# sz3/libcimbar

Hardware: NVIDIA H100
Metric: decoded cimbar frames/sec (1024x1024 mode-B) (higher is better)
Workload: dtype u8 (integer/bitwise; float32 only in the colour classifier, bit-exact vs reference)

## Files before the change

libcimbar_b200/csrc/k2_rs.cu:

```cuda
#include "cb200_common.cuh"
#include "k2_rs.cuh"
#include <cstring>
#include <cstdint>

namespace cb200 {

constexpr int kMaxParity = 64;

__constant__ uint8_t c_gf_exp[512];
__constant__ uint8_t c_gf_log[256];

__device__ __forceinline__ uint32_t slot_value(const uint8_t* __restrict__ cells, const uint16_t* __restrict__ idx,
                                               uint32_t s, int stream, int symbol_bits)
{
    uint32_t v = cells[idx[s]] & 0x7Fu;
    uint32_t sym_mask = (1u << symbol_bits) - 1u;
    if (stream == 0) return v & sym_mask;
    if (stream == 1) return v >> symbol_bits;
    return v;
}

__device__ __forceinline__ uint32_t stream_byte(const uint8_t* __restrict__ cells, const uint16_t* __restrict__ idx,
                                                uint32_t B, int w, int stream, int symbol_bits, uint32_t nslots)
{
    uint32_t bit0 = 8u * B;
    uint32_t s = bit0 / (uint32_t)w;
    uint32_t skip = bit0 - s * (uint32_t)w;
    uint32_t acc = 0, nbits = 0;
    while (nbits < skip + 8u) {
        uint32_t v = (s < nslots) ? slot_value(cells, idx, s, stream, symbol_bits) : 0u;
        acc = (acc << w) | v;
        nbits += (uint32_t)w;
        ++s;
    }
    return (acc >> (nbits - skip - 8u)) & 0xFFu;
}

__global__ void __launch_bounds__(256)
k_pack_raw(const Mode m, const uint8_t* __restrict__ cellvals, const uint16_t* __restrict__ idx, int n_frames,
           uint8_t* __restrict__ raw)
{
    int B = blockIdx.x * blockDim.x + threadIdx.x;
    int f = blockIdx.y;
    if (B >= m.cap_all || f >= n_frames) return;
    const uint8_t* cells = cellvals + (size_t)f * m.num_cells;
    uint32_t v;
    if (m.legacy) v = stream_byte(cells, idx, (uint32_t)B, m.symbol_bits + m.color_bits, 2, m.symbol_bits, (uint32_t)m.num_cells);
    else if (B < m.cap_sym) v = stream_byte(cells, idx, (uint32_t)B, m.symbol_bits, 0, m.symbol_bits, (uint32_t)m.num_cells);
    else v = stream_byte(cells, idx, (uint32_t)(B - m.cap_sym), m.color_bits, 1, m.symbol_bits, (uint32_t)m.num_cells);
    raw[(size_t)f * m.cap_all + B] = (uint8_t)v;
}

constexpr int kRsWarpsPerCta = 16;
constexpr int kLaDim = 40;
constexpr int kStagePitch = 196;

template <int T>
struct RsSmem {
    static constexpr bool kSynTable = false;
    static constexpr int GL = 8 * T;
    static constexpr int G = 32 / GL;
    uint8_t exp[512];
    uint8_t log[256];
    struct PerWarp {
        alignas(16) uint8_t stage[G * kStagePitch];
        alignas(4) uint8_t rem[64];
        alignas(2) uint16_t remlog[kMaxParity];
        uint8_t synd[kMaxParity];
        uint8_t loc[kMaxParity + 8];
        uint8_t last[kMaxParity + 8];
        uint8_t omega[kMaxParity];
        uint8_t roots[kMaxParity + 8];
    } w[kRsWarpsPerCta];
    uint8_t la[kLaDim][kLaDim];
};

template <class S>
__device__ __forceinline__ uint32_t gf_mul(const S& s, uint32_t a, uint32_t b)
{
    if (a == 0 || b == 0) return 0;
    return s.exp[(uint32_t)s.log[a] + (uint32_t)s.log[b]];
}
template <class S>
__device__ __forceinline__ uint32_t gf_div(const S& s, uint32_t a, uint32_t b)
{
    if (a == 0 || b == 0) return 0;
    return s.exp[255u + (uint32_t)s.log[a] - (uint32_t)s.log[b]];
}
__device__ __forceinline__ uint32_t lds_u32(uint32_t shared_addr)
{
    uint32_t v;
    asm("ld.shared.u32 %0, [%1];" : "=r"(v) : "r"(shared_addr));
    return v;
}
__device__ __forceinline__ uint32_t warp_xor(uint32_t v)
{
#pragma unroll
    for (int o = 16; o > 0; o >>= 1) v ^= __shfl_xor_sync(0xffffffffu, v, o);
    return v;
}

template <int T, class S, class W>
__device__ __forceinline__ bool rs_correct_block(const S& s, W& w, uint8_t* enc, const int md, const int blk, const int pad,
                                                 const bool holds, const uint32_t word, const int k, const int lane)
{
            __syncwarp();
            if (holds) reinterpret_cast<uint32_t*>(w.rem)[k] = word;
            __syncwarp();
            if constexpr (S::kSynTable) {
                if (lane < md) {
                    const uint32_t rb = w.rem[pad + lane];
                    w.masks[lane] = make_uint2((((rb & 15u) * 0x00204081u) & 0x01010101u) * 0xFFu, (((rb >> 4) * 0x00204081u) & 0x01010101u) * 0xFFu);
                }
                __syncwarp();
                uint32_t ax = 0, ay = 0;
#pragma unroll 6
                for (int i = 0; i < md; ++i) {
                    const uint2 mk = w.masks[i];
                    const uint2 tw = s.wsyn[i][lane];
                    ax ^= tw.x & mk.x; ay ^= tw.y & mk.y;
                }
                uint32_t x = ax ^ ay;
                x ^= x >> 16; x ^= x >> 8;
                if (lane < md) w.synd[lane] = (uint8_t)x;
            } else {
            for (int i = lane; i < md; i += 32) { const uint32_t rb = w.rem[pad + i]; w.remlog[i] = (uint16_t)(rb | ((uint32_t)s.log[rb] << 8)); }
            __syncwarp();
#pragma unroll
            for (int q = 0; q < T; ++q) {
                const int j = lane + 32 * q;
                if (j < md) {
                    uint32_t acc = 0;
#pragma unroll 6
                    for (int i = 0; i < md; ++i) {
                        const uint32_t rl = w.remlog[i];
                        const uint32_t t = s.exp[(rl >> 8) + (uint32_t)s.la[i][j]];
                        acc ^= (rl & 0xFFu) ? t : 0u;
                    }
                    w.synd[j] = (uint8_t)acc;
                }
            }
            }
            __syncwarp();
        uint32_t numerrors = 0, loc_order = 0, last_order = 0, last_disc = 1, delay = 1;
        if (T == 1) {
            uint32_t loc = (lane == 0), last = (lane == 0), lloc = 0;
            const uint32_t syn = (lane < md) ? (uint32_t)w.synd[lane] : 0u;
            const uint32_t spk = syn | ((uint32_t)s.log[syn] << 8);
            for (uint32_t i = 0; i < (uint32_t)md; ++i) {
                const uint32_t p = __shfl_sync(0xffffffffu, spk, (int)(i - (uint32_t)lane) & 31);
                uint32_t term = 0;
                if ((uint32_t)lane <= numerrors && loc != 0 && (p & 0xFFu) != 0) term = s.exp[lloc + (p >> 8)];
                const uint32_t disc = __reduce_xor_sync(0xffffffffu, term);
                if (disc == 0) { delay++; continue; }
                const uint32_t lscale = 255u + (uint32_t)s.log[disc] - (uint32_t)s.log[last_disc];
                const uint32_t top = last_order + delay;
                const uint32_t shifted = __shfl_up_sync(0xffffffffu, last, delay);
                const uint32_t lsc = lscale >= 255u ? lscale - 255u : lscale;
                const uint32_t sh = ((uint32_t)lane >= delay && (uint32_t)lane <= top && shifted != 0) ? (uint32_t)s.exp[(uint32_t)s.log[shifted] + lsc] : 0u;
                if (2 * numerrors <= i) {
                    if ((uint32_t)lane <= top) { const uint32_t t0 = loc; loc ^= sh; last = t0; }
                    lloc = s.log[loc];
                    const uint32_t tmp = loc_order;
                    loc_order = top; last_order = tmp;
                    numerrors = i + 1 - numerrors;
                    last_disc = disc;
                    delay = 1;
                    continue;
                }
                loc ^= sh;
                lloc = s.log[loc];
                if (top > loc_order) loc_order = top;
                delay++;
            }
            w.loc[lane] = (uint8_t)loc;
            if (lane < 8) w.loc[32 + lane] = 0;
            __syncwarp();
        } else {
        for (int j = lane; j < kMaxParity + 8; j += 32) { w.loc[j] = (j == 0); w.last[j] = (j == 0); }
        __syncwarp();
        for (uint32_t i = 0; i < (uint32_t)md; ++i) {
            uint32_t part = 0;
            for (uint32_t j = 1 + lane; j <= numerrors; j += 32) part ^= gf_mul(s, w.loc[j], w.synd[i - j]);
            uint32_t disc = warp_xor(part) ^ w.synd[i];
            if (disc == 0) { delay++; continue; }
            if (2 * numerrors <= i) {
                uint32_t top = last_order + delay;
                uint32_t sh[3], lc[3];
                int q = 0;
                for (uint32_t j = lane; j <= top; j += 32, ++q) {
                    sh[q] = (j < delay) ? 0u : gf_div(s, gf_mul(s, w.last[j - delay], disc), last_disc);
                    lc[q] = w.loc[j];
                }
                __syncwarp();
                q = 0;
                for (uint32_t j = lane; j <= top; j += 32, ++q) {
                    w.loc[j] = (uint8_t)(lc[q] ^ sh[q]);
                    w.last[j] = (uint8_t)lc[q];
                }
                __syncwarp();
                uint32_t tmp = loc_order;
                loc_order = top; last_order = tmp;
                numerrors = i + 1 - numerrors;
                last_disc = disc;
                delay = 1;
                continue;
            }
            for (uint32_t j = lane; j <= last_order; j += 32)
                w.loc[j + delay] ^= (uint8_t)gf_div(s, gf_mul(s, w.last[j], disc), last_disc);
            __syncwarp();
            if (last_order + delay > loc_order) loc_order = last_order + delay;
            delay++;
        }
        }
        const uint32_t order = loc_order;

        uint32_t myroots = 0;
        for (int k = 0; k < 8; ++k) {
            uint32_t e = (uint32_t)lane * 8u + (uint32_t)k;
            if (e == 0) continue;
            uint32_t le = s.log[e];
            uint32_t acc = w.loc[order];
            for (int i = (int)order - 1; i >= 0; --i) {
                uint32_t t = acc ? (uint32_t)s.exp[(uint32_t)s.log[acc] + le] : 0u;
                acc = t ^ w.loc[i];
            }
            if (acc == 0) myroots |= 1u << k;
        }
        uint32_t cnt = __popc(myroots);
        uint32_t incl = cnt;
#pragma unroll
        for (int o = 1; o < 32; o <<= 1) { uint32_t v = __shfl_up_sync(0xffffffffu, incl, o); if (lane >= o) incl += v; }
        uint32_t total = __shfl_sync(0xffffffffu, incl, 31);
        if (total != order || order == 0) {
            if (order == 0 && total == 0) {
            }
            return false;
        }
        {
            uint32_t pos = incl - cnt;
            for (int k = 0; k < 8; ++k) if (myroots & (1u << k)) w.roots[pos++] = (uint8_t)(lane * 8 + k);
        }
        for (int k = lane; k < md; k += 32) {
            uint32_t acc = 0;
            int lim = (int)order < k ? (int)order : k;
            for (int i = 0; i <= lim; ++i) acc ^= gf_mul(s, w.loc[i], w.synd[k - i]);
            w.omega[k] = (uint8_t)acc;
        }
        __syncwarp();
        for (uint32_t q = 0; q < order; ++q) {
            const uint32_t X = w.roots[q];
            const uint32_t lx = s.log[X];
            uint32_t tn = 0, td = 0;
#pragma unroll
            for (int qq = 0; qq < T; ++qq) {
                const uint32_t i = (uint32_t)lane + 32u * (uint32_t)qq;
                const uint32_t ex = (i * lx) % 255u;
                if (i < (uint32_t)md) { const uint32_t o = w.omega[i]; if (o) tn ^= s.exp[(uint32_t)s.log[o] + ex]; }
                if (i < order && (i & 1u) == 0u) { const uint32_t c = w.loc[i + 1]; if (c) td ^= s.exp[(uint32_t)s.log[c] + ex]; }
            }
            const uint32_t num = __reduce_xor_sync(0xffffffffu, tn), den = __reduce_xor_sync(0xffffffffu, td);
            const uint32_t err = gf_div(s, num, den);
            const uint32_t inv = s.exp[510u - lx];
            const uint32_t location = s.log[inv];
            if (lane == 0 && location >= (uint32_t)md && location < (uint32_t)blk)
                enc[blk - 1 - (int)location] ^= (uint8_t)err;
        }
        __syncwarp();
        return true;
}

template <int T, bool FUSED>
__global__ void __launch_bounds__(kRsWarpsPerCta * 32, (T == 1 ? 4 : 2))
k_rs_decode(const Mode m, const uint8_t* __restrict__ raw, const uint8_t* __restrict__ cellvals, const uint16_t* __restrict__ idx,
            int n_frames, int b_begin, int b_count, uint8_t* __restrict__ data_out, uint8_t* __restrict__ block_ok,
            const uint8_t* __restrict__ rho)
{
    using Smem = RsSmem<T>;
    constexpr int GL = Smem::GL, G = Smem::G;
    extern __shared__ __align__(16) uint8_t rs_smem_raw[];
    Smem& s = *reinterpret_cast<Smem*>(rs_smem_raw);
    uint32_t* lt = reinterpret_cast<uint32_t*>(rs_smem_raw + ((sizeof(Smem) + 127) & ~size_t(127)));
    const int tid = threadIdx.x, warp = tid >> 5, lane = tid & 31;
    for (int i = tid; i < 512; i += blockDim.x) s.exp[i] = c_gf_exp[i];
    for (int i = tid; i < 256; i += blockDim.x) s.log[i] = c_gf_log[i];
    __syncthreads();
    for (int e = tid; e < m.ecc_bytes * kLaDim; e += blockDim.x) {
        const int kk = e / kLaDim, j = e % kLaDim;
        s.la[kk][j] = (uint8_t)((255 - ((j + 1) * (m.ecc_bytes - kk)) % 255) % 255);
    }
    for (int e = tid; e < 4 * 256 * GL; e += blockDim.x) {
        const int j = e / (256 * GL), v = (e / GL) & 255, k = e % GL;
        uint32_t word = 0;
#pragma unroll
        for (int bb = 0; bb < 4; ++bb) word |= gf_mul(s, (uint32_t)v, (uint32_t)rho[j * 64 + 4 * k + bb]) << (8 * bb);
        lt[e] = word;
    }
    __syncthreads();

    const int md = m.ecc_bytes, blk = m.ecc_block, msg_len = m.msg_len;
    const int Pw = (md + 3) >> 2, pad = 4 * Pw - md, lead = (4 - (blk & 3)) & 3, nsteps = (lead + blk) >> 2;
    const long total_blocks = (long)n_frames * b_count;
    const long total_units = (total_blocks + G - 1) / G;
    typename Smem::PerWarp& w = s.w[warp];
    const int grp = lane / GL, k = lane % GL;
    const uint32_t lt_lane = (uint32_t)__cvta_generic_to_shared(lt) + 4u * (uint32_t)k;
    const uint32_t stage_lane = (uint32_t)__cvta_generic_to_shared(w.stage) + (uint32_t)(grp * kStagePitch);

    for (long unit = (long)blockIdx.x * kRsWarpsPerCta + warp; unit < total_units; unit += (long)gridDim.x * kRsWarpsPerCta) {
        __syncwarp();
#pragma unroll 1
        for (int g = 0; g < G; ++g) {
            const long gb = unit * G + g;
            uint8_t* st = w.stage + g * kStagePitch;
            if (lane < lead) st[lane] = 0;
            if (gb >= total_blocks) { for (int i = lane; i < blk; i += 32) st[lead + i] = 0; continue; }
            const int f = (int)(gb / b_count), b = b_begin + (int)(gb - (long)f * b_count);
            uint8_t* enc = st + lead;
            if (FUSED) {
                const uint8_t* cells = cellvals + (size_t)f * m.num_cells;
                const bool fast = !m.legacy && m.symbol_bits == 4 && m.color_bits == 2 && blk <= 160;
                if (fast) {
                    const uint32_t B0 = (uint32_t)b * (uint32_t)blk;
                    constexpr int kU = 5;
                    if ((int)B0 < m.cap_sym) {
                        uint32_t sl[kU];
#pragma unroll
                        for (int u = 0; u < kU; ++u) {
                            const int i = lane + 32 * u;
                            sl[u] = i < blk ? *reinterpret_cast<const uint32_t*>(idx + 2u * (B0 + (uint32_t)i)) : 0u;
                        }
                        uint32_t c0[kU], c1[kU];
#pragma unroll
                        for (int u = 0; u < kU; ++u) {
                            const int i = lane + 32 * u;
                            if (i < blk) { c0[u] = cells[sl[u] & 0xFFFFu]; c1[u] = cells[sl[u] >> 16]; } else { c0[u] = c1[u] = 0; }
                        }
#pragma unroll
                        for (int u = 0; u < kU; ++u) {
                            const int i = lane + 32 * u;
                            if (i < blk) enc[i] = (uint8_t)(((c0[u] & 15u) << 4) | (c1[u] & 15u));
                        }
                    } else {
                        uint2 sl[kU];
#pragma unroll
                        for (int u = 0; u < kU; ++u) {
                            const int i = lane + 32 * u;
                            sl[u] = i < blk ? *reinterpret_cast<const uint2*>(idx + 4u * (B0 + (uint32_t)i - (uint32_t)m.cap_sym)) : make_uint2(0u, 0u);
                        }
                        uint32_t c0[kU], c1[kU], c2[kU], c3[kU];
#pragma unroll
                        for (int u = 0; u < kU; ++u) {
                            const int i = lane + 32 * u;
                            if (i < blk) { c0[u] = cells[sl[u].x & 0xFFFFu]; c1[u] = cells[sl[u].x >> 16]; c2[u] = cells[sl[u].y & 0xFFFFu]; c3[u] = cells[sl[u].y >> 16]; }
                            else { c0[u] = c1[u] = c2[u] = c3[u] = 0; }
                        }
#pragma unroll
                        for (int u = 0; u < kU; ++u) {
                            const int i = lane + 32 * u;
                            if (i < blk)
                                enc[i] = (uint8_t)((((c0[u] >> 4) & 3u) << 6) | (((c1[u] >> 4) & 3u) << 4) | (((c2[u] >> 4) & 3u) << 2) | ((c3[u] >> 4) & 3u));
                        }
                    }
                } else {
                    for (int i = lane; i < blk; i += 32) {
                        uint32_t B = (uint32_t)b * (uint32_t)blk + (uint32_t)i, v;
                        if (m.legacy) v = stream_byte(cells, idx, B, m.symbol_bits + m.color_bits, 2, m.symbol_bits, (uint32_t)m.num_cells);
                        else if ((int)B < m.cap_sym) v = stream_byte(cells, idx, B, m.symbol_bits, 0, m.symbol_bits, (uint32_t)m.num_cells);
                        else v = stream_byte(cells, idx, B - (uint32_t)m.cap_sym, m.color_bits, 1, m.symbol_bits, (uint32_t)m.num_cells);
                        enc[i] = (uint8_t)v;
                    }
                }
            } else {
                const uint8_t* enc_g = raw + (size_t)f * m.cap_all + (size_t)b * blk;
                for (int i = lane; i < blk; i += 32) enc[i] = enc_g[i];
            }
        }
        __syncwarp();

        uint32_t word = 0;
        {
            const int top_src = grp * GL + (Pw - 1);
#pragma unroll 2
            for (int t = 0; t < nsteps; ++t) {
                const uint32_t ew = lds_u32(stage_lane + 4u * (uint32_t)t);
                const uint32_t tw = __shfl_sync(0xffffffffu, word, top_src);
                const uint32_t v = tw ^ __byte_perm(ew, 0u, 0x0123);
                const uint32_t r0 = lds_u32(lt_lane + (((v) & 0xFFu) + 0u) * (4u * GL));
                const uint32_t r1 = lds_u32(lt_lane + (((v >> 8) & 0xFFu) + 256u) * (4u * GL));
                const uint32_t r2 = lds_u32(lt_lane + (((v >> 16) & 0xFFu) + 512u) * (4u * GL));
                const uint32_t r3 = lds_u32(lt_lane + ((v >> 24) + 768u) * (4u * GL));
                uint32_t prev = __shfl_up_sync(0xffffffffu, word, 1, GL);
                if (k == 0) prev = 0;
                word = prev ^ r0 ^ r1 ^ r2 ^ r3;
            }
        }
        const uint32_t dirty = __ballot_sync(0xffffffffu, k < Pw && word != 0u);

#pragma unroll 1
        for (int g = 0; g < G; ++g) {
            const long gb = unit * G + g;
            if (gb >= total_blocks) break;
            const int f = (int)(gb / b_count), b = b_begin + (int)(gb - (long)f * b_count);
            uint8_t* out = data_out + ((size_t)f * m.nblocks + b) * msg_len;
            uint8_t* enc = w.stage + g * kStagePitch + lead;
            if (((dirty >> (g * GL)) & ((1u << GL) - 1u)) == 0u) {
                for (int i = lane; i < msg_len; i += 32) out[i] = enc[i];
                if (lane == 0) block_ok[(size_t)f * m.nblocks + b] = 1;
                continue;
            }
            __syncwarp();
            const bool good = rs_correct_block<T>(s, w, enc, md, blk, pad, grp == g && k < Pw, word, k, lane);
            __syncwarp();
            if (!good) {
                for (int i = lane; i < msg_len; i += 32) out[i] = 0;
                if (lane == 0) block_ok[(size_t)f * m.nblocks + b] = 0;
                continue;
            }
        for (int i = lane; i < msg_len; i += 32) out[i] = enc[i];
        if (lane == 0) block_ok[(size_t)f * m.nblocks + b] = 1;
        }
    }
}

constexpr int kFrWarps = 32;
constexpr int kFrFrames = 2;
constexpr int kFrBlk = 155, kFrWords = 39, kFrPitch = 160;

struct RsFrSmem {
    static constexpr bool kSynTable = true;
    uint8_t exp[512];
    uint8_t log[256];
    struct PerWarp {
        alignas(8) uint2 masks[32];
        alignas(4) uint8_t rem[64];
        alignas(2) uint16_t remlog[kMaxParity];
        uint8_t synd[kMaxParity];
        uint8_t loc[kMaxParity + 8];
        uint8_t last[kMaxParity + 8];
        uint8_t omega[kMaxParity];
        uint8_t roots[kMaxParity + 8];
    } w[kFrWarps];
    uint8_t la[kLaDim][kLaDim];
    alignas(8) uint2 wsyn[32][32];
};

__device__ __forceinline__ void cp_async16(uint32_t dst_shared, const void* src)
{
    asm volatile("cp.async.cg.shared.global [%0], [%1], 16;" ::"r"(dst_shared), "l"(src) : "memory");
}

__global__ void __launch_bounds__(kFrWarps * 32, 2)
k_rs_frames(const Mode m, const uint8_t* __restrict__ cellvals, const uint16_t* __restrict__ idx, int n_frames,
            uint8_t* __restrict__ data_out, uint8_t* __restrict__ block_ok, const uint8_t* __restrict__ rho, int cell_pitch)
{
    constexpr int GL = 8, G = 4;
    extern __shared__ __align__(16) uint8_t rs_smem_raw[];
    RsFrSmem& s = *reinterpret_cast<RsFrSmem*>(rs_smem_raw);
    uint8_t* dyn = rs_smem_raw + ((sizeof(RsFrSmem) + 127) & ~size_t(127));
    uint32_t* lt = reinterpret_cast<uint32_t*>(dyn);
    uint8_t* cellbuf = dyn + sizeof(uint32_t) * 4 * 256 * GL;
    uint8_t* rows = cellbuf + (size_t)kFrFrames * cell_pitch;
    const int tid = threadIdx.x, warp = tid >> 5, lane = tid & 31;
    const int md = m.ecc_bytes, msg_len = m.msg_len, nb = m.nblocks, upf = nb / G;
    const int Pw = (md + 3) >> 2, pad = 4 * Pw - md;
    const int words_per_frame = nb * kFrWords, sym_rows = m.cap_sym / kFrBlk, cell_vecs = m.num_cells >> 4;
    const bool coupled6 = m.legacy != 0;
    const int n_groups = (n_frames + kFrFrames - 1) / kFrFrames;
    const uint32_t cellbuf_s = (uint32_t)__cvta_generic_to_shared(cellbuf);

    auto load_cells = [&](int gi) {
        for (int fs = 0; fs < kFrFrames; ++fs) {
            const int f = gi * kFrFrames + fs;
            if (f >= n_frames) break;
            const uint8_t* src = cellvals + (size_t)f * m.num_cells;
            for (int i = tid; i < cell_vecs; i += (int)blockDim.x) cp_async16(cellbuf_s + (uint32_t)(fs * cell_pitch + 16 * i), src + 16 * i);
        }
        asm volatile("cp.async.commit_group;" ::: "memory");
    };
    int gi = blockIdx.x;
    if (gi < n_groups) load_cells(gi);

    for (int i = tid; i < 512; i += blockDim.x) s.exp[i] = c_gf_exp[i];
    for (int i = tid; i < 256; i += blockDim.x) s.log[i] = c_gf_log[i];
    __syncthreads();
    for (int e = tid; e < md * kLaDim; e += blockDim.x) {
        const int kk = e / kLaDim, j = e % kLaDim;
        s.la[kk][j] = (uint8_t)((255 - ((j + 1) * (md - kk)) % 255) % 255);
    }
    for (int e = tid; e < 32 * 32; e += blockDim.x) {
        const int i = e >> 5, j = e & 31;
        uint2 t = make_uint2(0u, 0u);
        if (i < md && j < md) {
            const uint32_t l = (uint32_t)((255 - ((j + 1) * (md - i)) % 255) % 255);
            t.x = (uint32_t)s.exp[l] | ((uint32_t)s.exp[l + 1] << 8) | ((uint32_t)s.exp[l + 2] << 16) | ((uint32_t)s.exp[l + 3] << 24);
            t.y = (uint32_t)s.exp[l + 4] | ((uint32_t)s.exp[l + 5] << 8) | ((uint32_t)s.exp[l + 6] << 16) | ((uint32_t)s.exp[l + 7] << 24);
        }
        s.wsyn[i][j] = t;
    }
    for (int e = tid; e < 4 * 256 * GL; e += blockDim.x) {
        const int v = e / (4 * GL), j = (e / GL) & 3, kk = e % GL;
        uint32_t word = 0;
#pragma unroll
        for (int bb = 0; bb < 4; ++bb) word |= gf_mul(s, (uint32_t)v, (uint32_t)rho[j * 64 + 4 * kk + bb]) << (8 * bb);
        lt[e] = word;
    }

    RsFrSmem::PerWarp& w = s.w[warp];
    const int grp = lane / GL, k = lane % GL;
    const uint32_t lt_lane = (uint32_t)__cvta_generic_to_shared(lt) + 4u * (uint32_t)k;
    const uint32_t vsel = 0x3210u ^ (0x1111u * (uint32_t)grp);
    const uint32_t lt0 = lt_lane + 32u * (uint32_t)(0 ^ grp), lt1 = lt_lane + 32u * (uint32_t)(1 ^ grp);
    const uint32_t lt2 = lt_lane + 32u * (uint32_t)(2 ^ grp), lt3 = lt_lane + 32u * (uint32_t)(3 ^ grp);

    for (; gi < n_groups; gi += gridDim.x) {
        asm volatile("cp.async.wait_all;" ::: "memory");
        __syncthreads();
        const int nf = (n_frames - gi * kFrFrames) < kFrFrames ? (n_frames - gi * kFrFrames) : kFrFrames;

        for (int wi = tid; wi < nf * words_per_frame; wi += (int)blockDim.x) {
            const int fs = wi >= words_per_frame ? 1 : 0;
            const int rem = wi - fs * words_per_frame;
            const int r = rem / kFrWords, q = rem - r * kFrWords;
            const uint8_t* cb = cellbuf + fs * cell_pitch;
            uint32_t b0, b1, b2, b3;
            if (coupled6) {
                auto byte6 = [&](const int B) -> uint32_t {
                    const uint32_t bit0 = 8u * (uint32_t)B, sl = bit0 / 6u, skip = bit0 - 6u * sl;
                    const uint32_t v0 = cb[idx[sl]] & 63u, v1 = cb[idx[sl + 1]] & 63u;
                    return (((v0 << 6) | v1) >> (4u - skip)) & 0xFFu;
                };
                const int B0 = r * kFrBlk + 4 * q - 1;
                b0 = q ? byte6(B0) : 0u; b1 = byte6(B0 + 1); b2 = byte6(B0 + 2); b3 = byte6(B0 + 3);
            } else if (r < sym_rows) {
                const uint32_t* ix = reinterpret_cast<const uint32_t*>(idx) + (r * kFrBlk + 4 * q);
                const uint32_t i0 = q ? ix[-1] : ix[0], i1 = ix[0], i2 = ix[1], i3 = ix[2];
                b0 = ((cb[i0 & 0xFFFFu] & 15u) << 4) | (cb[i0 >> 16] & 15u);
                b1 = ((cb[i1 & 0xFFFFu] & 15u) << 4) | (cb[i1 >> 16] & 15u);
                b2 = ((cb[i2 & 0xFFFFu] & 15u) << 4) | (cb[i2 >> 16] & 15u);
                b3 = ((cb[i3 & 0xFFFFu] & 15u) << 4) | (cb[i3 >> 16] & 15u);
            } else {
                const uint2* ix = reinterpret_cast<const uint2*>(idx) + ((r - sym_rows) * kFrBlk + 4 * q);
                const uint2 i0 = q ? ix[-1] : ix[0], i1 = ix[0], i2 = ix[1], i3 = ix[2];
                auto pack = [&](const uint2 ii) {
                    return (((uint32_t)cb[ii.x & 0xFFFFu] >> 4) & 3u) << 6 | (((uint32_t)cb[ii.x >> 16] >> 4) & 3u) << 4 |
                           (((uint32_t)cb[ii.y & 0xFFFFu] >> 4) & 3u) << 2 | (((uint32_t)cb[ii.y >> 16] >> 4) & 3u);
                };
                b0 = pack(i0); b1 = pack(i1); b2 = pack(i2); b3 = pack(i3);
            }
            if (q == 0) b0 = 0;
            *reinterpret_cast<uint32_t*>(rows + (size_t)(fs * nb + r) * kFrPitch + 4 * q) = b0 | (b1 << 8) | (b2 << 16) | (b3 << 24);
        }
        __syncthreads();
        if (gi + (int)gridDim.x < n_groups) load_cells(gi + (int)gridDim.x);

        if (warp >= nf * upf) continue;
        const int fs = warp >= upf ? 1 : 0, u = warp - fs * upf, f = gi * kFrFrames + fs;
        uint8_t* urow = rows + (size_t)(fs * nb + G * u) * kFrPitch;

        uint32_t word = 0;
        {
            const uint32_t stage_lane = (uint32_t)__cvta_generic_to_shared(urow) + (uint32_t)(grp * kFrPitch);
            const int top_src = grp * GL + (Pw - 1);
#pragma unroll 3
            for (int t = 0; t < kFrWords; ++t) {
                const uint32_t ew = lds_u32(stage_lane + 4u * (uint32_t)t);
                const uint32_t tw = __shfl_sync(0xffffffffu, word, top_src);
                const uint32_t v = __byte_perm(tw ^ __byte_perm(ew, 0u, 0x0123), 0u, vsel);
                const uint32_t r0 = lds_u32(lt0 + ((v) & 0xFFu) * 128u);
                const uint32_t r1 = lds_u32(lt1 + ((v >> 8) & 0xFFu) * 128u);
                const uint32_t r2 = lds_u32(lt2 + ((v >> 16) & 0xFFu) * 128u);
                const uint32_t r3 = lds_u32(lt3 + (v >> 24) * 128u);
                uint32_t prev = __shfl_up_sync(0xffffffffu, word, 1, GL);
                if (k == 0) prev = 0;
                word = prev ^ r0 ^ r1 ^ r2 ^ r3;
            }
        }
        const uint32_t dirty = __ballot_sync(0xffffffffu, k < Pw && word != 0u);
        uint32_t okflags = 0x01010101u;
        if (dirty) {
#pragma unroll 1
            for (int g = 0; g < G; ++g) {
                if (((dirty >> (g * GL)) & ((1u << GL) - 1u)) == 0u) continue;
                uint8_t* enc = urow + g * kFrPitch + 1;
                __syncwarp();
                const bool good = rs_correct_block<1>(s, w, enc, md, kFrBlk, pad, grp == g && k < Pw, word, k, lane);
                __syncwarp();
                if (!good) {
                    for (int i = lane; i < msg_len; i += 32) enc[i] = 0;
                    okflags &= ~(1u << (8 * g));
                }
            }
            __syncwarp();
        }
        uint32_t* out32 = reinterpret_cast<uint32_t*>(data_out + ((size_t)f * nb + (size_t)(G * u)) * msg_len);
        const uint32_t urow_s = (uint32_t)__cvta_generic_to_shared(urow);
        for (int wq = lane; wq < msg_len; wq += 32) {
            const int B = 4 * wq;
            int g = (B >= msg_len) + (B >= 2 * msg_len) + (B >= 3 * msg_len);
            int i = B - g * msg_len;
            uint32_t val;
            if (i + 4 <= msg_len) {
                const uint32_t a = (uint32_t)(g * kFrPitch + 1 + i);
                const uint32_t w0 = lds_u32(urow_s + (a & ~3u)), w1 = lds_u32(urow_s + (a & ~3u) + 4u);
                val = __funnelshift_r(w0, w1, 8u * (a & 3u));
            } else {
                val = 0;
#pragma unroll
                for (int j = 0; j < 4; ++j) {
                    val |= (uint32_t)urow[g * kFrPitch + 1 + i] << (8 * j);
                    if (++i == msg_len) { i = 0; ++g; }
                }
            }
            out32[wq] = val;
        }
        if (lane == 0) *reinterpret_cast<uint32_t*>(block_ok + (size_t)f * nb + (size_t)(G * u)) = okflags;
    }
}

__global__ void k_chunk_mask(const Mode m, const uint8_t* __restrict__ block_ok, int n_frames, uint32_t* __restrict__ mask)
{
    int f = blockIdx.x * blockDim.x + threadIdx.x;
    if (f >= n_frames) return;
    const uint8_t* ok = block_ok + (size_t)f * m.nblocks;
    uint32_t out = 0;
    bool carry = false;
    for (int q = 0; q < m.chunks_per_frame; ++q) {
        bool all = true;
        for (int k = 0; k < m.blocks_per_chunk; ++k) all = all && (ok[q * m.blocks_per_chunk + k] != 0);
        if (all && !carry) out |= 1u << q;
        carry = ok[q * m.blocks_per_chunk + m.blocks_per_chunk - 1] == 0;
    }
    mask[f] = out;
}

cudaError_t k2_init_tables(const uint8_t* exp512, const uint8_t* log256)
{
    cudaError_t e = cudaMemcpyToSymbol(c_gf_exp, exp512, 512);
    if (e != cudaSuccess) return e;
    return cudaMemcpyToSymbol(c_gf_log, log256, 256);
}

cudaError_t k2_pack_launch(const Mode& m, const uint8_t* d_cellvals, const uint16_t* d_idx, int n_frames, uint8_t* d_raw, cudaStream_t st)
{
    dim3 grid((m.cap_all + 255) / 256, n_frames);
    k_pack_raw<<<grid, 256, 0, st>>>(m, d_cellvals, d_idx, n_frames, d_raw); count_launch();
    return cudaGetLastError();
}

template <int T, bool FUSED>
static cudaError_t rs_launch_t(const Mode& m, const uint8_t* d_raw, const uint8_t* d_cellvals, const uint16_t* d_idx, int n_frames,
                               uint8_t* d_data, uint8_t* d_ok, const uint8_t* d_rho, int sm_count, cudaStream_t st, int b_begin = 0, int b_count = -1)
{
    if (b_count < 0) b_count = m.nblocks;
    if (m.ecc_block + 4 > kStagePitch || m.ecc_bytes > 8 * T * 4 || m.ecc_bytes > kLaDim) return cudaErrorInvalidValue;
    const size_t smem = ((sizeof(RsSmem<T>) + 127) & ~size_t(127)) + sizeof(uint32_t) * 4 * 256 * 8 * T;
    {
        cudaError_t e = cudaFuncSetAttribute(k_rs_decode<T, FUSED>, cudaFuncAttributeMaxDynamicSharedMemorySize, (int)smem);
        if (e != cudaSuccess) return e;
    }
    const int G = 4 / T;
    long total = (long)n_frames * b_count;
    long units = (total + G - 1) / G;
    long ctas = (units + kRsWarpsPerCta - 1) / kRsWarpsPerCta;
    long max_ctas = (long)sm_count * (T == 1 ? 4 : 2);
    if (ctas > max_ctas) ctas = max_ctas;
    if (ctas < 1) ctas = 1;
    k_rs_decode<T, FUSED><<<(int)ctas, kRsWarpsPerCta * 32, smem, st>>>(m, d_raw, d_cellvals, d_idx, n_frames, b_begin, b_count, d_data, d_ok, d_rho); count_launch();
    return cudaGetLastError();
}

cudaError_t k2_rs_launch(const Mode& m, const uint8_t* d_raw, int n_frames, uint8_t* d_data, uint8_t* d_ok, const uint8_t* d_rho, int sm_count, cudaStream_t st)
{
    if (m.ecc_bytes <= 32) return rs_launch_t<1, false>(m, d_raw, nullptr, nullptr, n_frames, d_data, d_ok, d_rho, sm_count, st);
    return rs_launch_t<2, false>(m, d_raw, nullptr, nullptr, n_frames, d_data, d_ok, d_rho, sm_count, st);
}

cudaError_t k2_rs_fused_launch(const Mode& m, const uint8_t* d_cellvals, const uint16_t* d_idx, int n_frames, uint8_t* d_data,
                               uint8_t* d_ok, const uint8_t* d_rho, int sm_count, cudaStream_t st, int b_begin, int b_count)
{
    if (b_count < 0) b_count = m.nblocks;
    const bool whole = b_begin == 0 && b_count == m.nblocks;
    const bool bits_ok = m.symbol_bits == 4 && m.color_bits == 2 && (!m.legacy || (size_t)m.num_cells * 6 == (size_t)m.cap_all * 8);
    if (whole && bits_ok && m.ecc_block == kFrBlk && m.ecc_bytes <= 32 &&
        m.ecc_bytes <= kLaDim && m.nblocks % 4 == 0 && kFrFrames * (m.nblocks / 4) <= kFrWarps && m.num_cells % 16 == 0 &&
        m.cap_sym % kFrBlk == 0 && (m.nblocks * m.msg_len) % 4 == 0 && ((uintptr_t)d_data & 3u) == 0 && n_frames > 0) {
        const int cell_pitch = m.num_cells;
        const size_t smem = ((sizeof(RsFrSmem) + 127) & ~size_t(127)) + sizeof(uint32_t) * 4 * 256 * 8 +
                            (size_t)kFrFrames * cell_pitch + (size_t)kFrFrames * m.nblocks * kFrPitch;
        if (smem <= 113 * 1024) {
            cudaError_t e = cudaFuncSetAttribute(k_rs_frames, cudaFuncAttributeMaxDynamicSharedMemorySize, (int)smem);
            if (e != cudaSuccess) return e;
            int groups = (n_frames + kFrFrames - 1) / kFrFrames, ctas = groups < 2 * sm_count ? groups : 2 * sm_count;
            k_rs_frames<<<ctas, 32 * kFrFrames * (m.nblocks / 4), smem, st>>>(m, d_cellvals, d_idx, n_frames, d_data, d_ok, d_rho, cell_pitch); count_launch();
            return cudaGetLastError();
        }
    }
    if (m.ecc_bytes <= 32) return rs_launch_t<1, true>(m, nullptr, d_cellvals, d_idx, n_frames, d_data, d_ok, d_rho, sm_count, st, b_begin, b_count);
    return rs_launch_t<2, true>(m, nullptr, d_cellvals, d_idx, n_frames, d_data, d_ok, d_rho, sm_count, st, b_begin, b_count);
}

void k2_remainder_basis(const uint8_t* gen, int parity, const uint8_t* gexp512, const uint8_t* glog256, uint8_t* rho_out )
{
    const int Pw = (parity + 3) / 4, D = 4 * Pw, pad = D - parity;
    uint8_t G[72] = {0};
    for (int k = 0; k <= parity; ++k) G[pad + k] = gen[k];
    auto mul = [&](uint8_t x, uint8_t y) -> uint8_t { return (x && y) ? gexp512[glog256[x] + glog256[y]] : 0; };
    uint8_t r[64] = {0};
    r[0] = 1;
    for (int e = 1; e <= D + 3; ++e) {
        const uint8_t top = r[D - 1];
        for (int k = D - 1; k > 0; --k) r[k] = r[k - 1];
        r[0] = 0;
        if (top) for (int k = 0; k < D; ++k) r[k] ^= mul(top, G[k]);
        if (e >= D) { for (int k = 0; k < 64; ++k) rho_out[(e - D) * 64 + k] = k < D ? r[k] : 0; }
    }
}

cudaError_t k2_mask_launch(const Mode& m, const uint8_t* d_ok, int n_frames, uint32_t* d_mask, cudaStream_t st)
{
    k_chunk_mask<<<(n_frames + 127) / 128, 128, 0, st>>>(m, d_ok, n_frames, d_mask); count_launch();
    return cudaGetLastError();
}

}
```

Baseline: 946,200.

## Process two RS units per warp with 64-bit remainder table lookups

Halves the RS kernel's thread count so each warp computes the parity remainder for two 4-block units at once. Lanes now hold two remainder words each and read paired words from a wider 8-word lookup table with 64-bit shared loads. The row-building loop is restructured so each thread computes cell indices once and reuses them across frames in the group. A compile-time-gated phase-timestamp probe and a benchmark script are added. Fewer threads per CTA lower warp-level parallelism, and dirty blocks are corrected serially per unit, which may hurt latency hiding.

```diff
diff --git a/libcimbar_b200/csrc/k2_rs.cu b/libcimbar_b200/csrc/k2_rs.cu
--- a/libcimbar_b200/csrc/k2_rs.cu
+++ b/libcimbar_b200/csrc/k2_rs.cu
@@ -91,6 +91,12 @@
 {
     uint32_t v;
     asm("ld.shared.u32 %0, [%1];" : "=r"(v) : "r"(shared_addr));
+    return v;
+}
+__device__ __forceinline__ uint2 lds_u64(uint32_t shared_addr)
+{
+    uint2 v;
+    asm("ld.shared.v2.u32 {%0, %1}, [%2];" : "=r"(v.x), "=r"(v.y) : "r"(shared_addr));
     return v;
 }
 __device__ __forceinline__ uint32_t warp_xor(uint32_t v)
@@ -450,16 +456,33 @@
     asm volatile("cp.async.cg.shared.global [%0], [%1], 16;" ::"r"(dst_shared), "l"(src) : "memory");
 }
 
-__global__ void __launch_bounds__(kFrWarps * 32, 2)
+enum RsPhase { kPhTop = 0, kPhCells = 1, kPhRows = 2, kPhRem = 3, kPhDirty = 4, kPhStore = 5 };
+#ifdef CB200_RS_PHASES
+constexpr int kRsPhases = 6;
+__device__ unsigned long long* g_rs_phase_buf;
+__device__ int g_rs_phase_passes;
+__device__ __forceinline__ void rs_phase(int pass, int ph)
+{
+    unsigned long long* b = g_rs_phase_buf;
+    const int passes = g_rs_phase_passes;
+    if (pass < 0) pass = passes;
+    if (b == nullptr || (threadIdx.x & 31) != 0 || pass > passes) return;
+    b[(((size_t)blockIdx.x * (passes + 1) + pass) * kFrWarps + (threadIdx.x >> 5)) * kRsPhases + ph] = clock64();
+}
+#else
+__device__ __forceinline__ void rs_phase(int, int) {}
+#endif
+
+__global__ void __launch_bounds__(kFrWarps / 2 * 32, 2)
 k_rs_frames(const Mode m, const uint8_t* __restrict__ cellvals, const uint16_t* __restrict__ idx, int n_frames,
             uint8_t* __restrict__ data_out, uint8_t* __restrict__ block_ok, const uint8_t* __restrict__ rho, int cell_pitch)
 {
-    constexpr int GL = 8, G = 4;
+    constexpr int GL = 4, G = 4, TW = 8;
     extern __shared__ __align__(16) uint8_t rs_smem_raw[];
     RsFrSmem& s = *reinterpret_cast<RsFrSmem*>(rs_smem_raw);
     uint8_t* dyn = rs_smem_raw + ((sizeof(RsFrSmem) + 127) & ~size_t(127));
     uint32_t* lt = reinterpret_cast<uint32_t*>(dyn);
-    uint8_t* cellbuf = dyn + sizeof(uint32_t) * 4 * 256 * GL;
+    uint8_t* cellbuf = dyn + sizeof(uint32_t) * 4 * 256 * TW;
     uint8_t* rows = cellbuf + (size_t)kFrFrames * cell_pitch;
     const int tid = threadIdx.x, warp = tid >> 5, lane = tid & 31;
     const int md = m.ecc_bytes, msg_len = m.msg_len, nb = m.nblocks, upf = nb / G;
@@ -479,6 +502,7 @@
         asm volatile("cp.async.commit_group;" ::: "memory");
     };
     int gi = blockIdx.x;
+    rs_phase(-1, kPhTop);
     if (gi < n_groups) load_cells(gi);
 
     for (int i = tid; i < 512; i += blockDim.x) s.exp[i] = c_gf_exp[i];
@@ -498,8 +522,8 @@
         }
         s.wsyn[i][j] = t;
     }
-    for (int e = tid; e < 4 * 256 * GL; e += blockDim.x) {
-        const int v = e / (4 * GL), j = (e / GL) & 3, kk = e % GL;
+    for (int e = tid; e < 4 * 256 * TW; e += blockDim.x) {
+        const int v = e / (4 * TW), j = (e / TW) & 3, kk = e % TW;
         uint32_t word = 0;
 #pragma unroll
         for (int bb = 0; bb < 4; ++bb) word |= gf_mul(s, (uint32_t)v, (uint32_t)rho[j * 64 + 4 * kk + bb]) << (8 * bb);
@@ -508,115 +532,164 @@
 
     RsFrSmem::PerWarp& w = s.w[warp];
     const int grp = lane / GL, k = lane % GL;
-    const uint32_t lt_lane = (uint32_t)__cvta_generic_to_shared(lt) + 4u * (uint32_t)k;
-    const uint32_t vsel = 0x3210u ^ (0x1111u * (uint32_t)grp);
-    const uint32_t lt0 = lt_lane + 32u * (uint32_t)(0 ^ grp), lt1 = lt_lane + 32u * (uint32_t)(1 ^ grp);
-    const uint32_t lt2 = lt_lane + 32u * (uint32_t)(2 ^ grp), lt3 = lt_lane + 32u * (uint32_t)(3 ^ grp);
-
-    for (; gi < n_groups; gi += gridDim.x) {
+    const uint32_t lt_lane = (uint32_t)__cvta_generic_to_shared(lt) + 8u * (uint32_t)k;
+    const uint32_t rows_s = (uint32_t)__cvta_generic_to_shared(rows);
+    const uint32_t sw = (uint32_t)grp & 3u;
+    const uint32_t vsel = 0x3210u ^ (0x1111u * sw);
+    const uint32_t lt0 = lt_lane + 32u * (0u ^ sw), lt1 = lt_lane + 32u * (1u ^ sw);
+    const uint32_t lt2 = lt_lane + 32u * (2u ^ sw), lt3 = lt_lane + 32u * (3u ^ sw);
+
+    for (int pass = 0; gi < n_groups; gi += gridDim.x, ++pass) {
+        rs_phase(pass, kPhTop);
         asm volatile("cp.async.wait_all;" ::: "memory");
         __syncthreads();
+        if (pass == 0) rs_phase(-1, kPhCells);
+        rs_phase(pass, kPhCells);
         const int nf = (n_frames - gi * kFrFrames) < kFrFrames ? (n_frames - gi * kFrFrames) : kFrFrames;
 
-        for (int wi = tid; wi < nf * words_per_frame; wi += (int)blockDim.x) {
-            const int fs = wi >= words_per_frame ? 1 : 0;
-            const int rem = wi - fs * words_per_frame;
-            const int r = rem / kFrWords, q = rem - r * kFrWords;
-            const uint8_t* cb = cellbuf + fs * cell_pitch;
-            uint32_t b0, b1, b2, b3;
+        for (int wi = tid; wi < words_per_frame; wi += (int)blockDim.x) {
+            const int r = wi / kFrWords, q = wi - r * kFrWords;
+            uint8_t* row = rows + (size_t)r * kFrPitch + 4 * q;
             if (coupled6) {
-                auto byte6 = [&](const int B) -> uint32_t {
-                    const uint32_t bit0 = 8u * (uint32_t)B, sl = bit0 / 6u, skip = bit0 - 6u * sl;
-                    const uint32_t v0 = cb[idx[sl]] & 63u, v1 = cb[idx[sl + 1]] & 63u;
-                    return (((v0 << 6) | v1) >> (4u - skip)) & 0xFFu;
-                };
                 const int B0 = r * kFrBlk + 4 * q - 1;
-                b0 = q ? byte6(B0) : 0u; b1 = byte6(B0 + 1); b2 = byte6(B0 + 2); b3 = byte6(B0 + 3);
+                const int B0j0 = B0 + (q == 0);
+                uint32_t cc[4];
+#pragma unroll
+                for (int j = 0; j < 4; ++j) {
+                    const uint32_t sl = 8u * (uint32_t)(j ? B0 + j : B0j0) / 6u;
+                    cc[j] = (uint32_t)idx[sl] | ((uint32_t)idx[sl + 1] << 16);
+                }
+#pragma unroll 1
+                for (int fs = 0; fs < nf; ++fs) {
+                    const uint8_t* cb = cellbuf + fs * cell_pitch;
+                    uint32_t word = 0;
+#pragma unroll
+                    for (int j = 0; j < 4; ++j) {
+                        const uint32_t skip = (8u * (uint32_t)(j ? B0 + j : B0j0)) % 6u;
+                        const uint32_t v0 = cb[cc[j] & 0xFFFFu] & 63u, v1 = cb[cc[j] >> 16] & 63u;
+                        word |= ((((v0 << 6) | v1) >> (4u - skip)) & 0xFFu) << (8 * j);
+                    }
+                    if (q == 0) word &= ~0xFFu;
+                    *reinterpret_cast<uint32_t*>(row + (size_t)fs * nb * kFrPitch) = word;
+                }
             } else if (r < sym_rows) {
                 const uint32_t* ix = reinterpret_cast<const uint32_t*>(idx) + (r * kFrBlk + 4 * q);
                 const uint32_t i0 = q ? ix[-1] : ix[0], i1 = ix[0], i2 = ix[1], i3 = ix[2];
-                b0 = ((cb[i0 & 0xFFFFu] & 15u) << 4) | (cb[i0 >> 16] & 15u);
-                b1 = ((cb[i1 & 0xFFFFu] & 15u) << 4) | (cb[i1 >> 16] & 15u);
-                b2 = ((cb[i2 & 0xFFFFu] & 15u) << 4) | (cb[i2 >> 16] & 15u);
-                b3 = ((cb[i3 & 0xFFFFu] & 15u) << 4) | (cb[i3 >> 16] & 15u);
+#pragma unroll 1
+                for (int fs = 0; fs < nf; ++fs) {
+                    const uint8_t* cb = cellbuf + fs * cell_pitch;
+                    uint32_t b0 = ((cb[i0 & 0xFFFFu] & 15u) << 4) | (cb[i0 >> 16] & 15u);
+                    const uint32_t b1 = ((cb[i1 & 0xFFFFu] & 15u) << 4) | (cb[i1 >> 16] & 15u);
+                    const uint32_t b2 = ((cb[i2 & 0xFFFFu] & 15u) << 4) | (cb[i2 >> 16] & 15u);
+                    const uint32_t b3 = ((cb[i3 & 0xFFFFu] & 15u) << 4) | (cb[i3 >> 16] & 15u);
+                    if (q == 0) b0 = 0;
+                    *reinterpret_cast<uint32_t*>(row + (size_t)fs * nb * kFrPitch) = b0 | (b1 << 8) | (b2 << 16) | (b3 << 24);
+                }
             } else {
                 const uint2* ix = reinterpret_cast<const uint2*>(idx) + ((r - sym_rows) * kFrBlk + 4 * q);
                 const uint2 i0 = q ? ix[-1] : ix[0], i1 = ix[0], i2 = ix[1], i3 = ix[2];
-                auto pack = [&](const uint2 ii) {
-                    return (((uint32_t)cb[ii.x & 0xFFFFu] >> 4) & 3u) << 6 | (((uint32_t)cb[ii.x >> 16] >> 4) & 3u) << 4 |
-                           (((uint32_t)cb[ii.y & 0xFFFFu] >> 4) & 3u) << 2 | (((uint32_t)cb[ii.y >> 16] >> 4) & 3u);
-                };
-                b0 = pack(i0); b1 = pack(i1); b2 = pack(i2); b3 = pack(i3);
-            }
-            if (q == 0) b0 = 0;
-            *reinterpret_cast<uint32_t*>(rows + (size_t)(fs * nb + r) * kFrPitch + 4 * q) = b0 | (b1 << 8) | (b2 << 16) | (b3 << 24);
+#pragma unroll 1
+                for (int fs = 0; fs < nf; ++fs) {
+                    const uint8_t* cb = cellbuf + fs * cell_pitch;
+                    auto pack = [&](const uint2 ii) {
+                        return (((uint32_t)cb[ii.x & 0xFFFFu] >> 4) & 3u) << 6 | (((uint32_t)cb[ii.x >> 16] >> 4) & 3u) << 4 |
+                               (((uint32_t)cb[ii.y & 0xFFFFu] >> 4) & 3u) << 2 | (((uint32_t)cb[ii.y >> 16] >> 4) & 3u);
+                    };
+                    const uint32_t b0 = q ? pack(i0) : 0u;
+                    *reinterpret_cast<uint32_t*>(row + (size_t)fs * nb * kFrPitch) = b0 | (pack(i1) << 8) | (pack(i2) << 16) | (pack(i3) << 24);
+                }
+            }
         }
         __syncthreads();
+        rs_phase(pass, kPhRows);
         if (gi + (int)gridDim.x < n_groups) load_cells(gi + (int)gridDim.x);
 
-        if (warp >= nf * upf) continue;
-        const int fs = warp >= upf ? 1 : 0, u = warp - fs * upf, f = gi * kFrFrames + fs;
-        uint8_t* urow = rows + (size_t)(fs * nb + G * u) * kFrPitch;
-
-        uint32_t word = 0;
+        if (warp * 2 >= nf * upf) continue;
+        const uint32_t brow_s = rows_s + (uint32_t)(8 * warp + grp) * kFrPitch;
+
+        uint32_t w0 = 0, w1 = 0;
         {
-            const uint32_t stage_lane = (uint32_t)__cvta_generic_to_shared(urow) + (uint32_t)(grp * kFrPitch);
-            const int top_src = grp * GL + (Pw - 1);
+            const int top_src = grp * GL + ((Pw - 1) >> 1);
+            const bool top_hi = ((Pw - 1) & 1) != 0;
 #pragma unroll 3
             for (int t = 0; t < kFrWords; ++t) {
-                const uint32_t ew = lds_u32(stage_lane + 4u * (uint32_t)t);
-                const uint32_t tw = __shfl_sync(0xffffffffu, word, top_src);
+                const uint32_t ew = lds_u32(brow_s + 4u * (uint32_t)t);
+                const uint32_t tw = __shfl_sync(0xffffffffu, top_hi ? w1 : w0, top_src);
                 const uint32_t v = __byte_perm(tw ^ __byte_perm(ew, 0u, 0x0123), 0u, vsel);
-                const uint32_t r0 = lds_u32(lt0 + ((v) & 0xFFu) * 128u);
-                const uint32_t r1 = lds_u32(lt1 + ((v >> 8) & 0xFFu) * 128u);
-                const uint32_t r2 = lds_u32(lt2 + ((v >> 16) & 0xFFu) * 128u);
-                const uint32_t r3 = lds_u32(lt3 + (v >> 24) * 128u);
-                uint32_t prev = __shfl_up_sync(0xffffffffu, word, 1, GL);
+                const uint2 r0 = lds_u64(lt0 + __byte_perm(v, 0u, 0x4440) * 128u);
+                const uint2 r1 = lds_u64(lt1 + __byte_perm(v, 0u, 0x4441) * 128u);
+                const uint2 r2 = lds_u64(lt2 + __byte_perm(v, 0u, 0x4442) * 128u);
+                const uint2 r3 = lds_u64(lt3 + __byte_perm(v, 0u, 0x4443) * 128u);
+                uint32_t prev = __shfl_up_sync(0xffffffffu, w1, 1, GL);
                 if (k == 0) prev = 0;
-                word = prev ^ r0 ^ r1 ^ r2 ^ r3;
-            }
-        }
-        const uint32_t dirty = __ballot_sync(0xffffffffu, k < Pw && word != 0u);
-        uint32_t okflags = 0x01010101u;
-        if (dirty) {
+                w1 = w0 ^ r0.y ^ r1.y ^ r2.y ^ r3.y;
+                w0 = prev ^ r0.x ^ r1.x ^ r2.x ^ r3.x;
+            }
+        }
+        const uint32_t dirty = __ballot_sync(0xffffffffu, (2 * k < Pw && w0 != 0u) || (2 * k + 1 < Pw && w1 != 0u));
+        rs_phase(pass, kPhRem);
 #pragma unroll 1
-            for (int g = 0; g < G; ++g) {
-                if (((dirty >> (g * GL)) & ((1u << GL) - 1u)) == 0u) continue;
-                uint8_t* enc = urow + g * kFrPitch + 1;
+        for (int h = 0; h < 2; ++h) {
+            const int U = 2 * warp + h;
+            if (U >= nf * upf) break;
+            const int fs = U >= upf ? 1 : 0, u = U - fs * upf, f = gi * kFrFrames + fs;
+            uint8_t* urow = rows + (size_t)(G * U) * kFrPitch;
+            uint32_t okflags = 0x01010101u;
+            const uint32_t udirty = (dirty >> (16 * h)) & 0xFFFFu;
+            if (udirty) {
+#pragma unroll 1
+                for (int g = 0; g < G; ++g) {
+                    if (((udirty >> (g * GL)) & ((1u << GL) - 1u)) == 0u) continue;
+                    uint8_t* enc = urow + g * kFrPitch + 1;
+                    __syncwarp();
+                    if (grp == 4 * h + g) {
+                        if (2 * k < Pw) reinterpret_cast<uint32_t*>(w.rem)[2 * k] = w0;
+                        if (2 * k + 1 < Pw) reinterpret_cast<uint32_t*>(w.rem)[2 * k + 1] = w1;
+                    }
+                    const bool good = rs_correct_block<1>(s, w, enc, md, kFrBlk, pad, false, 0u, 0, lane);
+                    __syncwarp();
+                    if (!good) {
+                        for (int i = lane; i < msg_len; i += 32) enc[i] = 0;
+                        okflags &= ~(1u << (8 * g));
+                    }
+                }
                 __syncwarp();
-                const bool good = rs_correct_block<1>(s, w, enc, md, kFrBlk, pad, grp == g && k < Pw, word, k, lane);
-                __syncwarp();
-                if (!good) {
-                    for (int i = lane; i < msg_len; i += 32) enc[i] = 0;
-                    okflags &= ~(1u << (8 * g));
-                }
-            }
-            __syncwarp();
-        }
-        uint32_t* out32 = reinterpret_cast<uint32_t*>(data_out + ((size_t)f * nb + (size_t)(G * u)) * msg_len);
-        const uint32_t urow_s = (uint32_t)__cvta_generic_to_shared(urow);
-        for (int wq = lane; wq < msg_len; wq += 32) {
-            const int B = 4 * wq;
-            int g = (B >= msg_len) + (B >= 2 * msg_len) + (B >= 3 * msg_len);
-            int i = B - g * msg_len;
-            uint32_t val;
-            if (i + 4 <= msg_len) {
-                const uint32_t a = (uint32_t)(g * kFrPitch + 1 + i);
-                const uint32_t w0 = lds_u32(urow_s + (a & ~3u)), w1 = lds_u32(urow_s + (a & ~3u) + 4u);
-                val = __funnelshift_r(w0, w1, 8u * (a & 3u));
-            } else {
-                val = 0;
-#pragma unroll
-                for (int j = 0; j < 4; ++j) {
-                    val |= (uint32_t)urow[g * kFrPitch + 1 + i] << (8 * j);
-                    if (++i == msg_len) { i = 0; ++g; }
-                }
-            }
-            out32[wq] = val;
-        }
-        if (lane == 0) *reinterpret_cast<uint32_t*>(block_ok + (size_t)f * nb + (size_t)(G * u)) = okflags;
-    }
-}
+            }
+            rs_phase(pass, kPhDirty);
+            uint32_t* out32 = reinterpret_cast<uint32_t*>(data_out + ((size_t)f * nb + (size_t)(G * u)) * msg_len);
+            const uint32_t urow_s = rows_s + (uint32_t)(G * U) * kFrPitch;
+            for (int wq = lane; wq < msg_len; wq += 32) {
+                const int B = 4 * wq;
+                int g = (B >= msg_len) + (B >= 2 * msg_len) + (B >= 3 * msg_len);
+                int i = B - g * msg_len;
+                uint32_t val;
+                if (i + 4 <= msg_len) {
+                    const uint32_t a = (uint32_t)(g * kFrPitch + 1 + i);
+                    const uint32_t x0 = lds_u32(urow_s + (a & ~3u)), x1 = lds_u32(urow_s + (a & ~3u) + 4u);
+                    val = __funnelshift_r(x0, x1, 8u * (a & 3u));
+                } else {
+                    val = 0;
+#pragma unroll
+                    for (int j = 0; j < 4; ++j) {
+                        val |= (uint32_t)urow[g * kFrPitch + 1 + i] << (8 * j);
+                        if (++i == msg_len) { i = 0; ++g; }
+                    }
+                }
+                out32[wq] = val;
+            }
+            if (lane == 0) *reinterpret_cast<uint32_t*>(block_ok + (size_t)f * nb + (size_t)(G * u)) = okflags;
+        }
+        rs_phase(pass, kPhStore);
+    }
+}
+
+#ifdef CB200_RS_PHASES
+extern "C" int cb200_rs_phase_attach(unsigned long long* d_buf, int passes)
+{
+    if (cudaMemcpyToSymbol(g_rs_phase_buf, &d_buf, sizeof(d_buf)) != cudaSuccess) return -1;
+    return cudaMemcpyToSymbol(g_rs_phase_passes, &passes, sizeof(passes)) == cudaSuccess ? 0 : -1;
+}
+#endif
 
 __global__ void k_chunk_mask(const Mode m, const uint8_t* __restrict__ block_ok, int n_frames, uint32_t* __restrict__ mask)
 {
@@ -692,7 +765,7 @@
             cudaError_t e = cudaFuncSetAttribute(k_rs_frames, cudaFuncAttributeMaxDynamicSharedMemorySize, (int)smem);
             if (e != cudaSuccess) return e;
             int groups = (n_frames + kFrFrames - 1) / kFrFrames, ctas = groups < 2 * sm_count ? groups : 2 * sm_count;
-            k_rs_frames<<<ctas, 32 * kFrFrames * (m.nblocks / 4), smem, st>>>(m, d_cellvals, d_idx, n_frames, d_data, d_ok, d_rho, cell_pitch); count_launch();
+            k_rs_frames<<<ctas, 32 * (kFrFrames * m.nblocks / 8), smem, st>>>(m, d_cellvals, d_idx, n_frames, d_data, d_ok, d_rho, cell_pitch); count_launch();
             return cudaGetLastError();
         }
     }
diff --git a/libcimbar_b200/rs_bench.py b/libcimbar_b200/rs_bench.py
--- /dev/null
+++ b/libcimbar_b200/rs_bench.py
@@ -0,0 +1,166 @@
+import argparse
+import ctypes as C
+import json
+import os
+import subprocess
+import sys
+import tempfile
+
+import numpy as np
+
+import libcimbar_b200 as cb
+from libcimbar_b200 import build as cbuild
+
+PHASES = ["top", "cells", "rows", "remainder", "dirty", "store"]
+
+
+def card():
+    import torch
+    out = {"name": torch.cuda.get_device_name(), "power_limit_w": None}
+    try:
+        import pynvml
+        pynvml.nvmlInit()
+        h = pynvml.nvmlDeviceGetHandleByIndex(torch.cuda.current_device())
+        out["power_limit_w"] = pynvml.nvmlDeviceGetEnforcedPowerLimit(h) / 1000.0
+        out["sm_max_mhz"] = pynvml.nvmlDeviceGetMaxClockInfo(h, pynvml.NVML_CLOCK_SM)
+    except Exception:
+        pass
+    return out
+
+
+def build_phase_lib(tmp):
+    cbuild.build()
+    obj = os.path.join(tmp, "k2_rs.o")
+    lib = os.path.join(tmp, "libcb200.so")
+    subprocess.check_call([cbuild._nvcc()] + cbuild.NVCC_FLAGS + ["-DCB200_RS_PHASES", "-c", os.path.join(cbuild.CSRC, "k2_rs.cu"),
+                                                                   "-o", obj])
+    objs = [obj if s == "k2_rs.cu" else os.path.join(cbuild.OBJ, s[:-3] + ".o") for s in cbuild._sources()]
+    subprocess.check_call([cbuild._nvcc(), "-gencode", "arch=compute_90a,code=sm_90a", "-shared", "-o", lib] + objs + ["-ldl"])
+    return lib
+
+
+def make_frames(ctx, info, B, workload, dev):
+    import torch
+    g = torch.Generator(device=dev)
+    g.manual_seed(0xC1B4)
+    payload = torch.randint(0, 256, (B, info.data_bytes), dtype=torch.uint8, device=dev, generator=g)
+    cells = torch.empty((B, info.total_cells), dtype=torch.uint8, device=dev)
+    ctx.encode_cells_dev(payload.data_ptr(), B, cells.data_ptr())
+    if workload == "errors1pct":
+        k = info.total_cells // 100
+        pos = torch.rand((B, info.total_cells), device=dev, generator=g).argsort(dim=1)[:, :k]
+        nvals = 1 << (info.symbol_bits + info.color_bits)
+        delta = torch.randint(1, nvals, (B, k), dtype=torch.uint8, device=dev, generator=g)
+        cells.scatter_(1, pos, (cells.gather(1, pos) + delta) % nvals)
+    frames = torch.empty((B, info.image_size_y, info.image_size_x, 3), dtype=torch.uint8, device=dev)
+    ctx.render_frames_dev(cells.data_ptr(), B, frames.data_ptr())
+    del cells
+    return payload, frames
+
+
+def split(stamps, passes):
+    body = stamps[:, :passes].astype(np.int64)
+    top = body[:, :, 0, 0]
+    cells = body[:, :, 0, 1]
+    rows = body[:, :, 0, 2]
+    live = body[:, :, :, 5] != 0
+    ends = {p: np.where(live, body[:, :, :, i], 0).max(axis=2) for p, i in (("remainder", 3), ("dirty", 4), ("store", 5))}
+    used = (top != 0) & (rows != 0) & live.any(axis=2)
+    rem = np.where(live, body[:, :, :, 3] - body[:, :, :, 2], 0).max(axis=2)
+    dirty = np.where(live, body[:, :, :, 4] - body[:, :, :, 3], 0).max(axis=2)
+    store = np.where(live, body[:, :, :, 5] - body[:, :, :, 4], 0).max(axis=2)
+    out = {"wait_cells": (cells - top)[used], "row_build": (rows - cells)[used], "remainder_slowest_warp": rem[used],
+           "dirty_slowest_warp": dirty[used], "store_slowest_warp": store[used], "pass_total": (ends["store"] - top)[used]}
+    res = {k: float(v.mean()) for k, v in out.items()}
+    pro = stamps[:, passes, 0].astype(np.int64)
+    res["prologue_tables"] = float((pro[:, 1] - pro[:, 0]).mean())
+    res["passes_measured"] = int(used.sum())
+    last = np.where(stamps[:, :passes, :, 5] != 0, stamps[:, :passes, :, 5], 0).max(axis=(1, 2)).astype(np.int64)
+    res["cta_total"] = float((last - pro[:, 0]).mean())
+    return res
+
+
+def main():
+    ap = argparse.ArgumentParser(description=__doc__.split("\n")[0])
+    ap.add_argument("--frames", type=int, default=10000)
+    ap.add_argument("--launches", type=int, default=40)
+    ap.add_argument("--warmup", type=int, default=5)
+    ap.add_argument("--mode", type=int, default=68)
+    ap.add_argument("--workloads", default="clean,errors1pct")
+    ap.add_argument("--phases", action="store_true", help="build and run the variant with phase stamps (see above)")
+    args = ap.parse_args()
+
+    import torch
+    if not torch.cuda.is_available():
+        raise SystemExit("rs_bench: no CUDA device")
+    tmp = None
+    if args.phases:
+        tmp = tempfile.TemporaryDirectory(prefix="cb200_rs_phases_")
+        cb.LIB_PATH = build_phase_lib(tmp.name)
+    dev = torch.device("cuda", 0)
+    torch.cuda.set_device(0)
+    B = args.frames
+    ctx = cb.Context(args.mode, max_frames=B, device=0)
+    info = ctx.info
+    stream = torch.cuda.Stream(device=dev)
+    torch.cuda.set_stream(stream)
+    ctx.set_stream(stream.cuda_stream)
+    chunks = torch.empty((B, info.data_bytes), dtype=torch.uint8, device=dev)
+    mask = torch.empty(B, dtype=torch.int32, device=dev)
+    result = {"tool": "rs_bench", "mode": args.mode, "frames": B, "launches": args.launches, "card": card(),
+              "build": "phase stamps (-DCB200_RS_PHASES)" if args.phases else "normal", "workloads": {}}
+    for wl in args.workloads.split(","):
+        payload, frames = make_frames(ctx, info, B, wl, dev)
+        torch.cuda.synchronize()
+        ctx.set_timing(False)
+        for _ in range(args.warmup):
+            ctx.decode_chunks_dev(frames.data_ptr(), B, chunks.data_ptr(), mask.data_ptr())
+        torch.cuda.synchronize()
+        ctx.set_timing(True)
+        rs = []
+        for i in range(args.launches):
+            ctx.decode_chunks_dev(frames.data_ptr(), B, chunks.data_ptr(), mask.data_ptr())
+            if (i + 1) % 32 == 0 or i + 1 == args.launches:
+                torch.cuda.synchronize()
+                rs += [ctx.get_timing(j)[3] for j in range(min(32, args.launches - len(rs)))]
+        ctx.set_timing(False)
+        torch.cuda.synchronize()
+        r = {"rs_ms_mean": float(np.mean(rs)), "rs_ms_min": float(np.min(rs)), "rs_ms_max": float(np.max(rs))}
+        full = (1 << info.chunks_per_frame) - 1
+        r["chunks_equal_payload"] = bool(torch.equal(chunks, payload)) and bool((mask == full).all().item())
+        r["frames_complete"] = int((mask == full).sum().item())
+        if args.phases:
+            lib = cb.load_library()
+            sms = info.sm_count
+            groups = (B + 1) // 2
+            ctas = min(groups, 2 * sms)
+            passes = -(-groups // ctas)
+            buf = torch.zeros(ctas * (passes + 1) * 32 * len(PHASES), dtype=torch.int64, device=dev)
+            lib.cb200_rs_phase_attach.argtypes = [C.c_void_p, C.c_int]
+            assert lib.cb200_rs_phase_attach(buf.data_ptr(), passes) == 0
+            ctx.set_timing(True)
+            ctx.decode_chunks_dev(frames.data_ptr(), B, chunks.data_ptr(), mask.data_ptr())
+            torch.cuda.synchronize()
+            inst_ms = ctx.get_timing(0)[3]
+            ctx.set_timing(False)
+            assert lib.cb200_rs_phase_attach(None, 0) == 0
+            st = buf.view(ctas, passes + 1, 32, len(PHASES)).cpu().numpy()
+            sp = split(st, passes)
+            per_cycle_ms = inst_ms / sp["cta_total"] if sp["cta_total"] > 0 else 0.0
+            sp["instrumented_rs_ms"] = inst_ms
+            sp["ms_by_share"] = {k: sp[k] * passes * per_cycle_ms for k in ("wait_cells", "row_build", "remainder_slowest_warp",
+                                                                           "dirty_slowest_warp", "store_slowest_warp")}
+            sp["ms_by_share"]["prologue_tables"] = sp["prologue_tables"] * per_cycle_ms
+            sp["grid"] = {"ctas": ctas, "passes": passes}
+            r["phases_cycles"] = sp
+        result["workloads"][wl] = r
+        del frames, payload
+        torch.cuda.empty_cache()
+    ctx.close()
+    print(json.dumps(result))
+    if tmp is not None:
+        tmp.cleanup()
+
+
+if __name__ == "__main__":
+    sys.exit(main())
```

Result: no change. 955,200 (median of 6 runs) (+1.0%).
